# qiyunzhu/woltka

Measured on AMD Instinct MI355X. Metric: alignment records/sec classified, higher is better.
Workload: dtype u8; 1 GPU; synthetic SAM text of 50M reads x <=16 hits (10.50 GB) resident in HBM, 2M-node taxonomy, ranks phylum,genus,species: device tokenizer per 64 MB block + one weighted histogram per sample (the kernels of `woltka classify`, host link left out); records_per_gpu=250034804, reads_per_gpu=50000000

## Files before the change

### woltka_amd/csrc/wk_dtok_fused.hpp

```cpp
#pragma once
#include "wk_dtok.hpp"

namespace wk {

constexpr uint32_t kFzThreads = 512;
constexpr uint32_t kFzWaves = kFzThreads / kWave;
constexpr uint32_t kFzTile = 16384;
constexpr uint32_t kFzBack = 1024;
constexpr uint32_t kFzFwd = 3072;
constexpr uint32_t kFzWin = kFzTile + kFzBack + kFzFwd;
constexpr uint32_t kFzChunks = kFzWin / 16 + 1;
constexpr uint32_t kFzChunksPerWave = (kFzChunks + kFzWaves - 1) / kFzWaves;
constexpr uint32_t kFzRounds = (kFzChunksPerWave + kWave - 1) / kWave;
constexpr uint32_t kFzLines = 1024;
constexpr uint32_t kFzStreams = 4;
constexpr uint32_t kFzCap = 1024;
static_assert(kFzCap >= kFzLines, "a window's records fit an empty buffer");
static_assert(kFzWin + 32 < 65536, "window offsets fit 16 bits");
constexpr uint32_t kFzCarry = 256;

constexpr uint32_t kDtokSpill = 64;

struct FusedArgs {
    const unsigned char* text;
    uint32_t n;
    uint32_t open_end;
    uint32_t span;
    const struct DictSlot8* dict8;
    const uint4* names16;
    uint32_t dict_mask;
    const unsigned char* arena;
    uint2* unknown;
    uint32_t unknown_cap;
    DtokState* state;
    DtokState* host_state;
    const unsigned long long* backup_prev;
    unsigned long long* backup_next;
    uint32_t* host_seq;
    uint32_t seq;
    StreamSet streams;
    const int32_t* submap;
    uint32_t n_submap;
    uint32_t ablate;
};

static_assert(sizeof(DtokState) % 8 == 0, "the packed totals are aligned");
__device__ __forceinline__ unsigned long long* fz_totals(DtokState* state) { return reinterpret_cast<unsigned long long*>(state + 1); }

__global__ void dtok_fused_begin_kernel(unsigned long long* __restrict__ backup, const unsigned long long* __restrict__ cursor, DtokState* state) {
    if (threadIdx.x < (uint32_t)kMaxStreams) backup[threadIdx.x] = cursor[threadIdx.x];
    if (threadIdx.x == 0) {
        *state = DtokState{0u, 0u, 0ull, 0ull, 0ull, 0u, 0u};
        *fz_totals(state) = 0ull;
    }
}

template <int kCtrl, int kRowMask>
__device__ __forceinline__ uint32_t fz_dpp_add(uint32_t v) {
    return v + (uint32_t)__builtin_amdgcn_update_dpp(0, (int)v, kCtrl, kRowMask, 0xF, false);
}
__device__ __forceinline__ uint32_t fz_wave_scan(uint32_t v) {
    static_assert(kWave == 64, "four rows of sixteen lanes");
    v = fz_dpp_add<0x111, 0xF>(v);
    v = fz_dpp_add<0x112, 0xF>(v);
    v = fz_dpp_add<0x114, 0xF>(v);
    v = fz_dpp_add<0x118, 0xF>(v);
    v = fz_dpp_add<0x142, 0xA>(v);
    v = fz_dpp_add<0x143, 0xC>(v);
    return v;
}
__device__ __forceinline__ uint32_t fz_last_lane(uint32_t v) { return (uint32_t)__builtin_amdgcn_readlane((int)v, kWave - 1); }
__device__ __forceinline__ uint32_t fz_wave_sum(uint32_t v) { return fz_last_lane(fz_wave_scan(v)); }
__device__ __forceinline__ unsigned long long fz_first_lane64(unsigned long long v) {
    return ((unsigned long long)(uint32_t)__builtin_amdgcn_readfirstlane((int)(uint32_t)(v >> 32)) << 32) |
           (uint32_t)__builtin_amdgcn_readfirstlane((int)(uint32_t)v);
}
constexpr uint32_t kFzNlBits = 11, kFzNlMask = (1u << kFzNlBits) - 1u;
static_assert(kFzRounds == 3 && kWave * 16u <= kFzNlMask, "two fields of 11 bits");
static_assert(kFzChunksPerWave > 2u * kWave && (kFzChunksPerWave - 2u * kWave) * 16u < (1u << (32u - 2u * kFzNlBits)), "and one of 10");

__device__ __forceinline__ uint4 fz_load_stream(const unsigned char* p) {
    typedef uint32_t u32x4 __attribute__((ext_vector_type(4)));
    const u32x4 v = __builtin_nontemporal_load(reinterpret_cast<const u32x4*>(p));
    return make_uint4(v.x, v.y, v.z, v.w);
}
__device__ __forceinline__ unsigned long long fz_load64(const unsigned char* p) {
    unsigned long long w;
    __builtin_memcpy(&w, p, 8);
    return w;
}
__device__ __forceinline__ uint32_t fz_load32(const unsigned char* p) {
    uint32_t w;
    __builtin_memcpy(&w, p, 4);
    return w;
}
__device__ __forceinline__ unsigned long long fz_eq_bytes(unsigned long long w, unsigned char c) {
    const unsigned long long x = w ^ (0x0101010101010101ull * c);
    return ~(((x & 0x7F7F7F7F7F7F7F7Full) + 0x7F7F7F7F7F7F7F7Full) | x | 0x7F7F7F7F7F7F7F7Full);
}
__device__ __forceinline__ uint32_t fz_marks32(uint32_t w, uint32_t c4) {
    const uint32_t x = w ^ c4;
    return ~(((x & 0x7F7F7F7Fu) + 0x7F7F7F7Fu) | x | 0x7F7F7F7Fu);
}
__device__ __forceinline__ unsigned long long fz_low_bytes(unsigned long long w, uint32_t k) {
    return k >= 8u ? w : (w & ((1ull << (8u * k)) - 1ull));
}

__device__ __forceinline__ unsigned long long fz_hash(const unsigned char* p, uint32_t n) {
    unsigned long long h = 0xcbf29ce484222325ull ^ ((unsigned long long)n * 0x9E3779B97F4A7C15ull);
    while (n >= 8u) {
        h = (h ^ fz_load64(p)) * 0x100000001b3ull;
        h ^= h >> 29;
        p += 8;
        n -= 8u;
    }
    const unsigned long long v = n ? fz_low_bytes(fz_load64(p), n) : 0ull;
    h = (h ^ v) * 0x100000001b3ull;
    h ^= h >> 32;
    h *= 0x9E3779B97F4A7C15ull;
    return h ^ (h >> 29);
}

__device__ __forceinline__ bool fz_same(const unsigned char* x, const unsigned char* y, uint32_t n) {
    while (n >= 8u) {
        if (fz_load64(x) != fz_load64(y)) return false;
        x += 8;
        y += 8;
        n -= 8u;
    }
    return n == 0u || fz_low_bytes(fz_load64(x) ^ fz_load64(y), n) == 0ull;
}

struct FzProbe {
    unsigned long long hv, n0, n1;
    uint32_t h;
    uint2 slot;
};
__device__ __forceinline__ FzProbe fz_probe_begin(const FusedArgs& a, const unsigned char* name, uint32_t rn) {
    FzProbe p;
    p.hv = fz_hash(name, rn);
    p.n0 = p.n1 = 0ull;
    if (rn <= 15u) {
        p.n0 = fz_low_bytes(fz_load64(name), rn);
        p.n1 = (rn > 8u ? fz_low_bytes(fz_load64(name + 8), rn - 8u) : 0ull) | ((unsigned long long)rn << 56);
    }
    p.h = (uint32_t)p.hv & a.dict_mask;
    p.slot = reinterpret_cast<const uint2*>(a.dict8)[p.h];
    return p;
}
__device__ __forceinline__ int32_t fz_probe_end(const FusedArgs& a, FzProbe p, const unsigned char* name, uint32_t rn, uint32_t abs_off) {
    for (;;) {
        const int32_t id = (int32_t)p.slot.y;
        if (id < 0) break;
        if (p.slot.x == (uint32_t)(p.hv >> 32)) {
            const uint4 nm = a.names16[id];
            const unsigned long long s0 = ((unsigned long long)nm.y << 32) | nm.x, s1 = ((unsigned long long)nm.w << 32) | nm.z;
            if (rn <= 15u) {
                if (s0 == p.n0 && s1 == p.n1) return id;
            } else if ((nm.w >> 24) == 0xFFu) {
                const unsigned char* full = a.arena + nm.x;
                if (fz_load32(full) == rn && fz_same(name, full + 4, rn)) return id;
            }
        }
        p.h = (p.h + 1u) & a.dict_mask;
        p.slot = reinterpret_cast<const uint2*>(a.dict8)[p.h];
    }
    const uint32_t at = atomicAdd(&a.state->n_unknown, 1u);
    if (at < a.unknown_cap)
        a.unknown[at] = make_uint2(abs_off, rn);
    else
        atomicOr(&a.state->flags, kDtokUnknownFull);
    return kLineUnknown;
}

__device__ bool fz_starts_run_slow(const unsigned char* __restrict__ text, uint32_t at, const unsigned char* q, uint32_t qn) {
    uint32_t pos = at;
    while (pos > 0u) {
        const uint32_t e = pos - 1u;
        uint32_t s = e;
        while (s > 0u && text[s - 1u] != '\n') --s;
        uint32_t tab[3], nt = 0;
        for (uint32_t p = s; p < e && nt < 3u; ++p)
            if (text[p] == '\t') tab[nt++] = p;
        if (nt == 3u && !(tab[2] - tab[1] == 2u && text[tab[1] + 1u] == '*')) {
            if (tab[0] - s != qn) return true;
            for (uint32_t k = 0; k < qn; ++k)
                if (text[s + k] != q[k]) return true;
            return false;
        }
        pos = s;
    }
    return true;
}

constexpr uint32_t kFiSubj = (1u << 23) - 1u;
constexpr uint32_t kFiMateShift = 24;
constexpr uint32_t kFiMapped = 1u << 26;
constexpr uint32_t kFiStart = 1u << 27;
constexpr uint32_t kFiFirst = 1u << 28;
constexpr uint32_t kFiExcl = 1u << 29;
constexpr uint32_t kFiDropped = 1u << 30;
constexpr uint32_t kFiRead = kFiMapped | (3u << kFiMateShift);
constexpr uint32_t kFiKey = kFiRead | kFiSubj;
constexpr uint32_t kFzPad = 8;

__device__ __forceinline__ uint32_t fz_octet(uint32_t z_lo, uint32_t z_hi) { return (((z_lo >> 7) | (z_hi >> 3)) * 0x00204081u >> 21) & 255u; }

__device__ __forceinline__ uint32_t fz_newlines16(uint4 v) {
    return fz_octet(fz_marks32(v.x, 0x0A0A0A0Au), fz_marks32(v.y, 0x0A0A0A0Au)) | (fz_octet(fz_marks32(v.z, 0x0A0A0A0Au), fz_marks32(v.w, 0x0A0A0A0Au)) << 8);
}

__device__ __forceinline__ uint32_t fz_tabs32(const unsigned char* p) {
    unsigned long long w[4];
#pragma unroll
    for (uint32_t i = 0; i < 4; ++i) w[i] = fz_load64(p + 8u * i);
    uint32_t m = 0;
#pragma unroll
    for (uint32_t i = 0; i < 4; ++i)
        m |= fz_octet(fz_marks32((uint32_t)w[i], 0x09090909u), fz_marks32((uint32_t)(w[i] >> 32), 0x09090909u)) << (8u * i);
    return m;
}

__global__ void __launch_bounds__(kFzThreads) __attribute__((amdgpu_waves_per_eu(6, 6))) dtok_fused_kernel(FusedArgs a) {
    __shared__ __attribute__((aligned(16))) unsigned char txt[kFzChunks * 16 + 32];
    __shared__ uint16_t ls[kFzLines + 2];
    __shared__ uint16_t f_qn[kFzLines], f_rb[kFzLines], f_rn[kFzLines];
    __shared__ __attribute__((aligned(16))) uint32_t info_[kFzPad + kFzCarry + kFzLines + kFzPad + 8];
    __shared__ uint32_t carry[kFzCarry];
    __shared__ uint32_t rbuf[kFzStreams][kFzCap];
    __shared__ uint32_t rcnt[kFzStreams];
    __shared__ unsigned long long newc_packed;
    static_assert(kFzStreams <= 4 && kFzLines < 65536, "four 16-bit counts");
    __shared__ unsigned long long gbase[kFzStreams];
    __shared__ uint32_t wtot[kFzWaves];
    __shared__ unsigned long long gbase_out[kMaxStreams];
    __shared__ unsigned long long wg_totals;
    __shared__ uint32_t own[4];
    __shared__ uint32_t wg_flags;
    uint32_t* const info = info_ + kFzPad + kFzCarry;

    const uint32_t tid = threadIdx.x, lane = tid & (kWave - 1), wave = tid / kWave;
    const uint32_t n_streams = a.streams.n_streams;
    if (tid < kFzStreams) rcnt[tid] = 0u;
    if (tid == 0) newc_packed = 0ull;
    if (tid == 0) wg_flags = 0u;
    if (tid == 0) wg_totals = 0ull;
    uint32_t my_flags = 0, my_reads = 0, my_lines = 0;
    const uint32_t text_end = a.n + (a.open_end ? 1u : 0u);

    auto flush_all = [&](bool last) {
        __syncthreads();
        if (tid < n_streams) {
            const uint32_t cnt = (a.ablate & 64u) ? 0u : rcnt[tid];
            unsigned long long base = 0ull;
            if (cnt) {
                base = atomicAdd(&a.streams.cursor[tid], (unsigned long long)cnt);
                if (base + cnt > a.streams.cap) atomicOr(&wg_flags, kDtokSpill);
            }
            gbase[tid] = base;
        }
        __syncthreads();
        for (uint32_t k = 0; k < n_streams; ++k) {
            const uint32_t cnt = (a.ablate & 64u) ? 0u : rcnt[k];
            const unsigned long long base = gbase[k];
            for (uint32_t i = tid; i < cnt; i += kFzThreads)
                if (base + i < a.streams.cap) a.streams.out[k][base + i] = rbuf[k][i];
        }
        if (last) return;
        __syncthreads();
        if (tid < n_streams) rcnt[tid] = 0u;
        __syncthreads();
    };

    const uint32_t t0 = blockIdx.x * a.span;
    const uint32_t t1 = a.n - t0 > a.span ? t0 + a.span : a.n;
    const uint32_t span_w1 = (uint32_t)min((unsigned long long)t1 + kFzFwd, (unsigned long long)text_end);
    uint32_t wpos = t0 >= kFzBack ? t0 - kFzBack : 0u;
    uint32_t mode = 0u;
    uint32_t counted = t0;
    bool wide = false;
    uint32_t nc = 0u;
    uint32_t cq_pos = 0u, cq_len = 0u;
    const uint32_t max_trips = a.span / 16u + 2u;
    for (uint32_t trip = 0;; ++trip) {
        if (trip >= max_trips) {
            my_flags |= kDtokSpill;
            break;
        }
        const uint32_t w0 = wpos & ~15u;
        const uint32_t lead = wpos - w0;
        const uint32_t w1 = (uint32_t)min((mode == 0u ? (unsigned long long)t0 + kFzTile + kFzFwd : (unsigned long long)w0 + kFzWin),
                                           (unsigned long long)(wide ? text_end : span_w1));
        const bool to_end = w1 == text_end;
        const bool last_win = wide || w1 == span_w1;
        __syncthreads();
        if (tid < 3u) own[tid] = tid < 2u ? 0xFFFFFFFFu : 0u;
        if (tid < kFzPad) info[-(int32_t)nc - 1 - (int32_t)tid] = kFiStart;
        for (uint32_t i = tid; i < nc; i += kFzThreads) info[(int32_t)i - (int32_t)nc] = carry[i];

        uint4 v[kFzRounds];
#pragma unroll
        for (uint32_t r = 0; r < kFzRounds; ++r) {
            const uint32_t cw = r * kWave + lane;
            const uint32_t p = w0 + (wave * kFzChunksPerWave + cw) * 16u;
            v[r] = make_uint4(0u, 0u, 0u, 0u);
            if (cw < kFzChunksPerWave && p < a.n && p < w1) v[r] = fz_load_stream(a.text + p);
        }
        uint32_t marks[kFzRounds];
        uint32_t nl_packed = 0;
        const uint32_t in_lo = max(wpos, counted), in_hi = min(min(w1, a.n), t1);
        const uint32_t wave_c0 = (uint32_t)__builtin_amdgcn_readfirstlane((int)(wave * kFzChunksPerWave));
#pragma unroll
        for (uint32_t r = 0; r < kFzRounds; ++r) {
            const uint32_t cw = r * kWave + lane;
            const uint32_t c = wave * kFzChunksPerWave + cw;
            const uint32_t p = w0 + c * 16u;
            marks[r] = 0u;
            const uint32_t rc0 = wave_c0 + r * kWave, rp0 = w0 + rc0 * 16u;
            const bool interior = (r + 1u) * kWave <= kFzChunksPerWave && rc0 + kWave <= kFzChunks && rp0 >= in_lo &&
                                  (unsigned long long)rp0 + kWave * 16u <= in_hi;
            if (interior) {
                *reinterpret_cast<uint4*>(txt + c * 16u) = v[r];
                const uint32_t m = fz_newlines16(v[r]);
                const uint32_t cnt = (uint32_t)__popc(m);
                my_lines += cnt;
                marks[r] = m;
                nl_packed |= cnt << (kFzNlBits * r);
            } else if (cw < kFzChunksPerWave && c < kFzChunks) {
                *reinterpret_cast<uint4*>(txt + c * 16u) = v[r];
                if (p < w1) {
                    uint32_t m = fz_newlines16(v[r]);
                    if (p + 16u > a.n) m &= p >= a.n ? 0u : (1u << (a.n - p)) - 1u;
                    if (p >= counted && p < t1) my_lines += (uint32_t)__popc(m);
                    if (a.open_end && a.n >= p && a.n < p + 16u) m |= 1u << (a.n - p);
                    if (p + 16u > w1) m &= (1u << (w1 - p)) - 1u;
                    if (p < wpos) m &= ~((1u << (wpos - p)) - 1u);
                    marks[r] = m;
                    nl_packed |= (uint32_t)__popc(m) << (kFzNlBits * r);
                }
            }
        }
        const uint32_t nl_inc = fz_wave_scan(nl_packed);
        const uint32_t nl_wave = fz_last_lane(nl_inc);
        if (lane == 0) wtot[wave] = (nl_wave & kFzNlMask) + ((nl_wave >> kFzNlBits) & kFzNlMask) + (nl_wave >> (2u * kFzNlBits));
        __syncthreads();
        uint32_t before = 0, total_nl = 0;
#pragma unroll
        for (uint32_t w = 0; w < kFzWaves; ++w) {
            before += w < wave ? wtot[w] : 0u;
            total_nl += wtot[w];
        }
        const bool too_many = total_nl + 1u > kFzLines || (a.ablate & (32u | 512u));
        if (too_many) {
            if (!(a.ablate & 512u)) my_flags |= kDtokSpill;
        } else {
            if (tid == 0) ls[0] = (uint16_t)lead;
            uint32_t line = before;
#pragma unroll
            for (uint32_t r = 0; r < kFzRounds; ++r) {
                const uint32_t c = wave * kFzChunksPerWave + r * kWave + lane;
                uint32_t at = line + ((nl_inc >> (kFzNlBits * r)) & kFzNlMask) - (uint32_t)__popc(marks[r]);
                uint32_t m = marks[r];
                while (m) {
                    const uint32_t b = (uint32_t)__ffs((int)m) - 1u;
                    ls[++at] = (uint16_t)(c * 16u + b + 1u);
                    m &= m - 1u;
                }
                line += (nl_wave >> (kFzNlBits * r)) & kFzNlMask;
            }
        }
        __syncthreads();
        const uint32_t trail = too_many ? wpos : w0 + (uint32_t)__builtin_amdgcn_readfirstlane((int)(uint32_t)ls[total_nl]);
        if (!too_many && last_win && trail >= t0 && trail < t1) my_flags |= kDtokSpill;
        const uint32_t first_line = mode != 0u || w0 == 0u ? 0u : 1u;
        const uint32_t n_lines = too_many ? 0u : total_nl;
        if (tid < kFzPad) info[n_lines + tid] = kFiStart;
        if (tid == 0 && first_line) info[0] = 0u;

        for (uint32_t k = first_line + tid; k < n_lines; k += kFzThreads) {
            const uint32_t s = ls[k], e = (uint32_t)ls[k + 1] - 1u;
            uint32_t tab[3] = {0, 0, 0}, nt = 0;
            if (!(a.ablate & 256u)) {
                uint32_t m = fz_tabs32(txt + s);
                if (e - s < 32u) m &= (1u << (e - s)) - 1u;
                nt = min((uint32_t)__popc(m), 3u);
                tab[0] = s + (uint32_t)__ffs((int)m) - 1u;
                m &= m - 1u;
                tab[1] = s + (uint32_t)__ffs((int)m) - 1u;
                m &= m - 1u;
                tab[2] = s + (uint32_t)__ffs((int)m) - 1u;
                for (uint32_t p = s + 32u; nt < 3u && p < e; p += 32u) {
                    m = fz_tabs32(txt + p);
                    if (e - p < 32u) m &= (1u << (e - p)) - 1u;
                    for (; m && nt < 3u; m &= m - 1u) {
                        const uint32_t q = p + (uint32_t)__ffs((int)m) - 1u;
                        if (nt == 0u)
                            tab[0] = q;
                        else if (nt == 1u)
                            tab[1] = q;
                        else
                            tab[2] = q;
                        ++nt;
                    }
                }
            }
            uint32_t word = 0;
            if (a.ablate & 16u) {
            } else if (nt < 3u) {
                my_flags |= kDtokShortLine;
            } else {
                const uint32_t fl = tab[1] - tab[0] - 1u;
                const unsigned long long fw = fz_load64(txt + tab[0] + 1u);
                uint32_t flag = 0;
                bool digits = fl >= 1u && fl <= 6u;
                for (uint32_t i = 0; i < fl && i < 6u; ++i) {
                    const uint32_t d = ((uint32_t)(fw >> (8u * i)) & 0xFFu) - (uint32_t)'0';
                    digits &= d <= 9u;
                    flag = flag * 10u + d;
                }
                const uint32_t rb = tab[1] + 1u, rn = tab[2] - rb;
                if (!digits) {
                    my_flags |= kDtokShortLine;
                } else if (rn == 1u && txt[rb] == '*') {
                } else {
                    const uint32_t mate = (flag >> 6) & 3u;
                    if (mate == 3u) my_flags |= kDtokBothMates;
                    word = kFiMapped | (mate << kFiMateShift);
                    f_qn[k] = (uint16_t)(tab[0] - s);
                    f_rb[k] = (uint16_t)rb;
                    f_rn[k] = (uint16_t)rn;
                }
            }
            info[k] = word;
        }
        __syncthreads();

        for (uint32_t k = first_line + tid; k < n_lines; k += kFzThreads) {
            if (!(info[k] & kFiMapped) || w0 + ls[k] < t0) continue;
            const unsigned char* name = txt + f_rb[k];
            const uint32_t rn = f_rn[k];
            FzProbe probe;
            if (!(a.ablate & 1u)) probe = fz_probe_begin(a, name, rn);
            uint32_t j = k;
            bool found = false;
            while (j > first_line) {
                --j;
                if (info[j] & kFiMapped) {
                    found = true;
                    break;
                }
            }
            bool start;
            if (a.ablate & 8u)
                start = true;
            else if (found)
                start = f_qn[j] != f_qn[k] || !fz_same(txt + ls[k], txt + ls[j], f_qn[k]);
            else if (nc)
                start = f_qn[k] != cq_len || !fz_same(txt + ls[k], a.text + cq_pos, cq_len);
            else if (mode == 1u || wpos == 0u)
                start = true;
            else
                start = fz_starts_run_slow(a.text, w0 + ls[first_line], txt + ls[k], f_qn[k]);
            int32_t sid = (a.ablate & 1u) ? (int32_t)(fz_load32(name + 4) % 1000u) : fz_probe_end(a, probe, name, rn, w0 + f_rb[k]);
            bool excluded = false;
            if (a.submap && sid >= 0) {
                if ((uint32_t)sid < a.n_submap) {
                    sid = a.submap[sid];
                    if (sid == kLineExcluded) {
                        excluded = true;
                        sid = 0;
                    }
                } else {
                    my_flags |= kDtokSpill;
                    sid = -1;
                }
            }
            info[k] |= (start ? kFiStart : 0u) | (excluded ? kFiExcl : 0u) | (sid < 0 ? kFiSubj : ((uint32_t)sid & kFiSubj));
            if (start) {
                atomicMin(&own[w0 + ls[k] < t1 ? 0 : 1], k);
                atomicMax(&own[2], k);
            }
        }
        __syncthreads();
        const uint32_t o0 = (uint32_t)__builtin_amdgcn_readfirstlane((int)own[0]), o1 = (uint32_t)__builtin_amdgcn_readfirstlane((int)own[1]);
        const uint32_t last = (uint32_t)__builtin_amdgcn_readfirstlane((int)own[2]);
        const uint32_t lpos = w0 + (uint32_t)__builtin_amdgcn_readfirstlane((int)(uint32_t)ls[o0 != 0xFFFFFFFFu ? last : 0u]);
        const bool has_first = nc != 0u || o0 != 0xFFFFFFFFu;
        const int32_t first_own = nc ? -(int32_t)nc : (int32_t)o0;
        int32_t ka = 0, kb = 0;
        uint32_t next = 0u, next_mode = 0u, nc_next = 0u;
        bool more = false, again = false, put_aside = false;
        if (too_many) {
            if ((a.ablate & (32u | 512u)) && !last_win) {
                next = w1;
                next_mode = 2u;
                more = true;
            }
        } else if (o1 != 0xFFFFFFFFu) {
            kb = (int32_t)o1;
            ka = has_first ? first_own : kb;
        } else if (to_end) {
            kb = (int32_t)n_lines;
            ka = has_first ? first_own : kb;
        } else if (last_win && a.span <= kFzTile) {
            if (o0 != 0xFFFFFFFFu) my_flags |= kDtokSpill;
        } else if (o0 != 0xFFFFFFFFu && (nc != 0u || last != o0 || lpos > wpos)) {
            kb = (int32_t)last;
            ka = first_own;
            next = lpos;
            next_mode = 1u;
            more = true;
            again = last_win;
        } else if (o0 != 0xFFFFFFFFu && last_win && !wide) {
            next = wpos;
            next_mode = 1u;
            more = again = true;
        } else if (o0 != 0xFFFFFFFFu || nc != 0u) {
            put_aside = true;
        } else if (!last_win) {
            next = trail;
            next_mode = 2u;
            more = trail > wpos && trail < t1;
            if (trail <= wpos) my_flags |= kDtokSpill;
        }
        if (put_aside) {
            if (tid == 0) {
                uint32_t c = nc;
                for (uint32_t k = first_line; k < n_lines; ++k) {
                    const uint32_t w = info[k];
                    if (w & kFiMapped) {
                        if (c < kFzCarry) carry[c] = w & ~(kFiFirst | kFiDropped);
                        ++c;
                    }
                }
                own[3] = c;
            }
            __syncthreads();
            nc_next = (uint32_t)__builtin_amdgcn_readfirstlane((int)own[3]);
            if (nc_next > kFzCarry || trail <= wpos) {
                my_flags |= kDtokSpill;
                nc_next = 0u;
            } else {
                if (nc == 0u) {
                    cq_pos = wpos;
                    cq_len = (uint32_t)__builtin_amdgcn_readfirstlane((int)(uint32_t)f_qn[0]);
                }
                next = trail;
                next_mode = 2u;
                more = true;
                again = last_win;
            }
        }
        for (int32_t k = ka + (int32_t)tid; k < kb; k += (int32_t)kFzThreads) {
            const uint32_t mk = info[k];
            if (!(mk & kFiMapped)) continue;
            if (mk & kFiExcl) {
                int32_t j = k;
                while (!(info[j] & kFiStart)) --j;
                atomicOr(&info[j], kFiDropped);
                continue;
            }
            bool dup = false;
            if (!(mk & kFiStart) && !(a.ablate & 2u)) {
                bool done = false;
                for (int32_t j = k; !done; j -= 8) {
                    uint32_t w[8];
#pragma unroll
                    for (uint32_t i = 0; i < 8; ++i) w[i] = info[j - 1 - (int32_t)i];
#pragma unroll
                    for (uint32_t i = 0; i < 8; ++i) {
                        dup |= !done && ((w[i] ^ mk) & kFiKey) == 0u;
                        done |= (w[i] & kFiStart) != 0u;
                    }
                }
            }
            if (!dup) atomicOr(&info[k], kFiFirst);
        }
        __syncthreads();
        for (int32_t k0 = ka; k0 < kb; k0 += (int32_t)kFzThreads) {
            const int32_t k = k0 + (int32_t)tid;
            bool rec = false;
            uint32_t word = 0, sl = 0, at = 0;
            if (k < kb && (info[k] & kFiFirst) && !(a.ablate & 4u)) {
                const uint32_t mk = info[k];
                uint32_t pos = 0, size = 1;
                bool dropped = (mk & kFiStart) && (mk & kFiDropped);
                if (!(a.ablate & (2u | 128u))) {
                    if (!(mk & kFiStart)) {
                        bool done = false;
                        for (int32_t j = k; !done; j -= 8) {
                            uint32_t w[8];
#pragma unroll
                            for (uint32_t i = 0; i < 8; ++i) w[i] = info[j - 1 - (int32_t)i];
#pragma unroll
                            for (uint32_t i = 0; i < 8; ++i) {
                                pos += (!done && (w[i] & kFiFirst) && ((w[i] ^ mk) & kFiRead) == 0u) ? 1u : 0u;
                                dropped |= !done && (w[i] & kFiStart) && (w[i] & kFiDropped);
                                done |= (w[i] & kFiStart) != 0u;
                            }
                        }
                    }
                    bool done = false;
                    for (int32_t j = k + 1; !done; j += 8) {
                        uint32_t w[8];
#pragma unroll
                        for (uint32_t i = 0; i < 8; ++i) w[i] = info[j + (int32_t)i];
#pragma unroll
                        for (uint32_t i = 0; i < 8; ++i) {
                            done |= (w[i] & kFiStart) != 0u;
                            size += (!done && (w[i] & kFiFirst) && ((w[i] ^ mk) & kFiRead) == 0u) ? 1u : 0u;
                        }
                    }
                    size += pos;
                }
                if (size > (uint32_t)WK_WEIGHT_MAX_K) my_flags |= kDtokBigRead;
                const uint32_t s = mk & kFiSubj;
                if (s != kFiSubj && !dropped) {
                    rec = true;
                    word = s | ((pos & 15u) << kWordSubjBits) | ((size & 31u) << kWordSizeShift);
                    sl = s / kSliceBins;
                    if (sl >= n_streams) sl = n_streams - 1u;
                    my_reads += pos == 0u ? 1u : 0u;
                }
            }
            {
                unsigned long long add = 0;
                uint32_t mine_before = 0;
                for (uint32_t s2 = 0; s2 < n_streams; ++s2) {
                    const unsigned long long m = __ballot(rec && sl == s2);
                    add |= (unsigned long long)__popcll(m) << (16u * s2);
                    if (rec && sl == s2) mine_before = (uint32_t)__popcll(m & ((1ull << lane) - 1ull));
                }
                if (add) {
                    unsigned long long base = 0;
                    if (lane == 0) base = atomicAdd(&newc_packed, add);
                    base = fz_first_lane64(base);
                    at = (uint32_t)(base >> (16u * sl)) & 0xFFFFu;
                    at += mine_before;
                }
            }
            __syncthreads();
            const unsigned long long newc = newc_packed;
            bool full = false;
            for (uint32_t s2 = 0; s2 < n_streams; ++s2) full |= rcnt[s2] + ((uint32_t)(newc >> (16u * s2)) & 0xFFFFu) > kFzCap;
            if (full) flush_all(false);
            if (rec) rbuf[sl][rcnt[sl] + at] = word;
            __syncthreads();
            if (tid < n_streams) rcnt[tid] += (uint32_t)(newc >> (16u * tid)) & 0xFFFFu;
            if (tid == 0) newc_packed = 0ull;
            __syncthreads();
        }
        if (!more) break;
        wpos = next;
        mode = next_mode;
        wide = again;
        nc = nc_next;
        counted = w1;
    }
    if (my_flags) atomicOr(&wg_flags, my_flags);
    {
        const uint32_t reads_w = fz_wave_sum(my_reads), lines_w = fz_wave_sum(my_lines);
        const unsigned long long t = ((unsigned long long)lines_w << 32) | reads_w;
        if (lane == 0 && t) atomicAdd(&wg_totals, t);
    }
    flush_all(true);
    __syncthreads();
    if (tid == 0) {
        if (wg_totals) __hip_atomic_fetch_add(fz_totals(a.state), wg_totals, __ATOMIC_RELAXED, __HIP_MEMORY_SCOPE_AGENT);
        if (wg_flags) atomicOr(&a.state->flags, wg_flags);
        __threadfence();
        own[0] = atomicAdd(&a.state->done, 1u) == gridDim.x - 1u ? 1u : 0u;
    }
    __syncthreads();
    if (own[0]) {
        __threadfence();
        if (tid < (uint32_t)kMaxStreams) {
            const unsigned long long cur = __hip_atomic_load(&a.streams.cursor[tid], __ATOMIC_RELAXED, __HIP_MEMORY_SCOPE_AGENT);
            a.backup_next[tid] = cur;
            gbase_out[tid] = tid < n_streams ? cur - a.backup_prev[tid] : 0ull;
        }
        __syncthreads();
        if (tid == 0) {
            DtokState st{};
            st.flags = __hip_atomic_load(&a.state->flags, __ATOMIC_RELAXED, __HIP_MEMORY_SCOPE_AGENT);
            st.n_unknown = __hip_atomic_load(&a.state->n_unknown, __ATOMIC_RELAXED, __HIP_MEMORY_SCOPE_AGENT);
            const unsigned long long totals = __hip_atomic_load(fz_totals(a.state), __ATOMIC_RELAXED, __HIP_MEMORY_SCOPE_AGENT);
            for (uint32_t k = 0; k < (uint32_t)kMaxStreams; ++k) st.n_out += gbase_out[k];
            st.n_reads = totals & 0xFFFFFFFFull;
            st.n_lines = totals >> 32;
            *a.host_state = st;
            *a.state = DtokState{0u, 0u, 0ull, 0ull, 0ull, 0u, 0u};
            *fz_totals(a.state) = 0ull;
            __threadfence_system();
            if (a.host_seq) __hip_atomic_store(a.host_seq, a.seq, __ATOMIC_RELEASE, __HIP_MEMORY_SCOPE_SYSTEM);
        }
    }
}

}
```

Baseline: 14.23 billion records/s.

## Replace per-record linear scans with ballot-built bitplanes for read position and size

Each wave now ballots read-start bits and per-mate first-hit bits into shared-memory 64-bit planes, replacing the kFiFirst flag and its atomicOr. The record-emission pass computes each hit's position, read size and head line with popcount and clz/ctz over those planes, instead of walking info[] backward and forward 8 words at a time. The goal is to cut the shared-memory scan work that grows with hits per read. The cost is a small planes array in LDS (five planes of 20 words) and extra ballots in the dedup pass. The dropped flag is now read from the head line.

```diff
diff --git a/woltka_amd/csrc/wk_dtok_fused.hpp b/woltka_amd/csrc/wk_dtok_fused.hpp
--- a/woltka_amd/csrc/wk_dtok_fused.hpp
+++ b/woltka_amd/csrc/wk_dtok_fused.hpp
@@ -1,5 +1,6 @@
 #pragma once
 #include "wk_dtok.hpp"
+#include "wk_dtok_planes.hpp"
 
 namespace wk {
 
@@ -18,6 +19,7 @@
 static_assert(kFzCap >= kFzLines, "a window's records fit an empty buffer");
 static_assert(kFzWin + 32 < 65536, "window offsets fit 16 bits");
 constexpr uint32_t kFzCarry = 256;
+static_assert(kFzCarry + kFzLines <= kFpMaxLines && kFzThreads % kWave == 0, "a window's owned lines fit the planes, a wave's lines one word");
 
 constexpr uint32_t kDtokSpill = 64;
 
@@ -197,7 +199,6 @@
 constexpr uint32_t kFiMateShift = 24;
 constexpr uint32_t kFiMapped = 1u << 26;
 constexpr uint32_t kFiStart = 1u << 27;
-constexpr uint32_t kFiFirst = 1u << 28;
 constexpr uint32_t kFiExcl = 1u << 29;
 constexpr uint32_t kFiDropped = 1u << 30;
 constexpr uint32_t kFiRead = kFiMapped | (3u << kFiMateShift);
@@ -227,6 +228,7 @@
     __shared__ uint16_t f_qn[kFzLines], f_rb[kFzLines], f_rn[kFzLines];
     __shared__ __attribute__((aligned(16))) uint32_t info_[kFzPad + kFzCarry + kFzLines + kFzPad + 8];
     __shared__ uint32_t carry[kFzCarry];
+    __shared__ unsigned long long planes[kFpPlanes][kFpWords];
     __shared__ uint32_t rbuf[kFzStreams][kFzCap];
     __shared__ uint32_t rcnt[kFzStreams];
     __shared__ unsigned long long newc_packed;
@@ -374,7 +376,6 @@
         if (!too_many && last_win && trail >= t0 && trail < t1) my_flags |= kDtokSpill;
         const uint32_t first_line = mode != 0u || w0 == 0u ? 0u : 1u;
         const uint32_t n_lines = too_many ? 0u : total_nl;
-        if (tid < kFzPad) info[n_lines + tid] = kFiStart;
         if (tid == 0 && first_line) info[0] = 0u;
 
         for (uint32_t k = first_line + tid; k < n_lines; k += kFzThreads) {
@@ -529,7 +530,7 @@
                 for (uint32_t k = first_line; k < n_lines; ++k) {
                     const uint32_t w = info[k];
                     if (w & kFiMapped) {
-                        if (c < kFzCarry) carry[c] = w & ~(kFiFirst | kFiDropped);
+                        if (c < kFzCarry) carry[c] = w & ~kFiDropped;
                         ++c;
                     }
                 }
@@ -551,17 +552,17 @@
                 again = last_win;
             }
         }
-        for (int32_t k = ka + (int32_t)tid; k < kb; k += (int32_t)kFzThreads) {
-            const uint32_t mk = info[k];
-            if (!(mk & kFiMapped)) continue;
-            if (mk & kFiExcl) {
+        for (int32_t k0 = ka; k0 < kb; k0 += (int32_t)kFzThreads) {
+            const int32_t k = k0 + (int32_t)tid;
+            const uint32_t mk = k < kb ? info[k] : 0u;
+            const bool mapped = (mk & kFiMapped) != 0u, excl = mapped && (mk & kFiExcl);
+            if (excl) {
                 int32_t j = k;
                 while (!(info[j] & kFiStart)) --j;
                 atomicOr(&info[j], kFiDropped);
-                continue;
             }
             bool dup = false;
-            if (!(mk & kFiStart) && !(a.ablate & 2u)) {
+            if (mapped && !excl && !(mk & kFiStart) && !(a.ablate & 2u)) {
                 bool done = false;
                 for (int32_t j = k; !done; j -= 8) {
                     uint32_t w[8];
@@ -574,44 +575,34 @@
                     }
                 }
             }
-            if (!dup) atomicOr(&info[k], kFiFirst);
+            const bool first = mapped && !excl && !dup;
+            const uint32_t mate = (mk >> kFiMateShift) & 3u;
+            const uint32_t wi = (uint32_t)__builtin_amdgcn_readfirstlane((int)((uint32_t)(k0 - ka) / kWave + wave));
+            const bool put = lane == 0 && wi < kFpWords;
+            const unsigned long long p_start = __ballot(mapped && (mk & kFiStart));
+            if (put) planes[kFpStart][wi] = p_start;
+#pragma unroll
+            for (uint32_t m = 0; m < 4; ++m) {
+                const unsigned long long p_first = __ballot(first && mate == m);
+                if (put) planes[kFpFirst + m][wi] = p_first;
+            }
         }
         __syncthreads();
         for (int32_t k0 = ka; k0 < kb; k0 += (int32_t)kFzThreads) {
             const int32_t k = k0 + (int32_t)tid;
             bool rec = false;
             uint32_t word = 0, sl = 0, at = 0;
-            if (k < kb && (info[k] & kFiFirst) && !(a.ablate & 4u)) {
-                const uint32_t mk = info[k];
+            const uint32_t li = (uint32_t)(k - ka);
+            const uint32_t mk = k < kb ? info[k] : 0u;
+            const unsigned long long* const mine = planes[kFpFirst + ((mk >> kFiMateShift) & 3u)];
+            if (k < kb && ((mine[li / 64u] >> (li % 64u)) & 1ull) && !(a.ablate & 4u)) {
                 uint32_t pos = 0, size = 1;
                 bool dropped = (mk & kFiStart) && (mk & kFiDropped);
                 if (!(a.ablate & (2u | 128u))) {
-                    if (!(mk & kFiStart)) {
-                        bool done = false;
-                        for (int32_t j = k; !done; j -= 8) {
-                            uint32_t w[8];
-#pragma unroll
-                            for (uint32_t i = 0; i < 8; ++i) w[i] = info[j - 1 - (int32_t)i];
-#pragma unroll
-                            for (uint32_t i = 0; i < 8; ++i) {
-                                pos += (!done && (w[i] & kFiFirst) && ((w[i] ^ mk) & kFiRead) == 0u) ? 1u : 0u;
-                                dropped |= !done && (w[i] & kFiStart) && (w[i] & kFiDropped);
-                                done |= (w[i] & kFiStart) != 0u;
-                            }
-                        }
-                    }
-                    bool done = false;
-                    for (int32_t j = k + 1; !done; j += 8) {
-                        uint32_t w[8];
-#pragma unroll
-                        for (uint32_t i = 0; i < 8; ++i) w[i] = info[j + (int32_t)i];
-#pragma unroll
-                        for (uint32_t i = 0; i < 8; ++i) {
-                            done |= (w[i] & kFiStart) != 0u;
-                            size += (!done && (w[i] & kFiFirst) && ((w[i] ^ mk) & kFiRead) == 0u) ? 1u : 0u;
-                        }
-                    }
-                    size += pos;
+                    const FpRead r = fp_read(planes[kFpStart], mine, li, (uint32_t)(kb - ka));
+                    pos = r.pos;
+                    size = r.size;
+                    dropped = (info[ka + (int32_t)r.head] & kFiDropped) != 0u;
                 }
                 if (size > (uint32_t)WK_WEIGHT_MAX_K) my_flags |= kDtokBigRead;
                 const uint32_t s = mk & kFiSubj;
diff --git a/woltka_amd/csrc/wk_dtok_planes.hpp b/woltka_amd/csrc/wk_dtok_planes.hpp
--- /dev/null
+++ b/woltka_amd/csrc/wk_dtok_planes.hpp
@@ -0,0 +1,60 @@
+#pragma once
+#include <cstdint>
+
+#if defined(__HIPCC__) || defined(__CUDACC__)
+#define WK_FP_FN __host__ __device__ __forceinline__
+#else
+#define WK_FP_FN inline
+#endif
+
+namespace wk {
+
+constexpr uint32_t kFpMaxLines = 1280;
+constexpr uint32_t kFpWords = kFpMaxLines / 64;
+constexpr uint32_t kFpStart = 0, kFpFirst = 1;
+constexpr uint32_t kFpPlanes = 5;
+
+WK_FP_FN unsigned long long fp_upto(uint32_t b) { return ~0ull >> (63u - b); }
+
+WK_FP_FN uint32_t fp_head(const unsigned long long* s, uint32_t i) {
+    uint32_t w = i >> 6;
+    unsigned long long m = s[w] & fp_upto(i & 63u);
+    while (m == 0ull && w > 0u) m = s[--w];
+    return m ? w * 64u + 63u - (uint32_t)__builtin_clzll(m) : 0u;
+}
+
+WK_FP_FN uint32_t fp_end(const unsigned long long* s, uint32_t i, uint32_t n) {
+    const uint32_t words = (n + 63u) >> 6;
+    uint32_t w = i >> 6;
+    unsigned long long m = s[w] & ~fp_upto(i & 63u);
+    while (m == 0ull && ++w < words) m = s[w];
+    if (m == 0ull) return n;
+    const uint32_t e = w * 64u + (uint32_t)__builtin_ctzll(m);
+    return e < n ? e : n;
+}
+
+WK_FP_FN uint32_t fp_count(const unsigned long long* f, uint32_t lo, uint32_t hi) {
+    uint32_t c = 0u;
+    if (lo >= hi) return c;
+    const uint32_t last = hi - 1u;
+    for (uint32_t w = lo >> 6;; ++w) {
+        unsigned long long m = f[w];
+        if (w == lo >> 6) m &= ~0ull << (lo & 63u);
+        if (w == last >> 6) m &= fp_upto(last & 63u);
+        c += (uint32_t)__builtin_popcountll(m);
+        if (w == last >> 6) return c;
+    }
+}
+
+struct FpRead {
+    uint32_t head, pos, size;
+};
+WK_FP_FN FpRead fp_read(const unsigned long long* s, const unsigned long long* f, uint32_t i, uint32_t n) {
+    FpRead r;
+    r.head = fp_head(s, i);
+    r.pos = fp_count(f, r.head, i);
+    r.size = r.pos + fp_count(f, i, fp_end(s, i, n));
+    return r;
+}
+
+}
```

Result: faster. 15.01 billion records/s (median of 6 runs) (+5.5%).
